# unitaryfoundation/qrack

Measured on NVIDIA H100. Metric: gates/sec at 30q random circuit; Apply2x2 HBM GB/s vs roofline, higher is better.
Workload: dtype f32

## Files before the change

### include/b200sv.h

```cpp
#ifndef B200SV_H
#define B200SV_H

#include <stddef.h>
#include <stdint.h>

#ifdef __cplusplus
extern "C" {
#endif

#define B200SV_OK 0
#define B200SV_EINVAL (-1)
#define B200SV_ENOMEM (-2)
#define B200SV_ECUDA (-3)
#define B200SV_ESTATE (-4)

typedef struct b200sv_state* b200sv_t;

int b200sv_abi_version(void);
const char* b200sv_last_error(void);
int b200sv_device_count(int* count);
int b200sv_device_info(int dev, uint64_t* total_bytes, uint64_t* free_bytes, int* sm_count);
int b200sv_can_access_peer(int dev, int peer, int* can);

int b200sv_create(int device, int n_qubits, int precision, b200sv_t* out);
// ... 91 lines not shown
int b200sv_indexed(b200sv_t s, int kind, int index_start, int index_length, int value_start, int value_length,
    int carry_index, int carry_in, const unsigned char* values);
int b200sv_hash(b200sv_t s, int start, int length, const unsigned char* values);
int b200sv_phase_flip_if_less(b200sv_t s, uint64_t greater_perm, int start, int length, int flag_index);

int b200sv_apply_gates(b200sv_t s, int n_gates, const uint64_t* off1, const uint64_t* off2, const uint64_t* pmasks,
    const double* mats8);

int b200sv_emulate_fused(int n_qubits, int precision, int n_gates, const uint64_t* off1, const uint64_t* off2,
    const uint64_t* pmasks, const double* mats8, void* host_state);
int b200sv_plan_gates(int n_qubits, int precision, int n_gates, const uint64_t* off1, const uint64_t* off2,
    const uint64_t* pmasks, const double* mats8, int* n_sweeps, int* n_passes, int* n_ops);
int b200sv_emulate_fused_pull(int n_qubits, int precision, int n_gates, const uint64_t* off1, const uint64_t* off2,
    const uint64_t* pmasks, const double* mats8, int k, const int* victim_bits, int rank, void* const* src_states,
    void* out_state);

typedef struct b200sv_stats {
    uint64_t gates_submitted;
    uint64_t kernel_launches;
    uint64_t fused_sweeps;
    uint64_t fused_gates;
    uint64_t single_launches;
    uint64_t bytes_swept;
    uint64_t pull_sweeps;
} b200sv_stats;
int b200sv_get_stats(b200sv_t s, b200sv_stats* out);
int b200sv_reset_stats(b200sv_t s);

int b200sv_timer_begin(b200sv_t s);
int b200sv_timer_end(b200sv_t s, double* elapsed_ms);
int b200sv_flush_l2(b200sv_t s, uint64_t bytes);

#ifdef __cplusplus
}
#endif
#endif
```

### qrack_b200/_abi.py

```python
from __future__ import annotations

import ctypes
import os
import subprocess
from ctypes import POINTER, c_char_p, c_double, c_int, c_uint64, c_void_p

_HERE = os.path.dirname(os.path.abspath(__file__))
LIB_PATH = os.environ.get("B200SV_LIB") or os.path.join(_HERE, "libb200sv.so")
CSRC = os.path.join(_HERE, "csrc")
SOURCES = ["b200sv.cu", "fused.cu"]
NVCC_FLAGS = ["-gencode", "arch=compute_90a,code=sm_90a", "-lineinfo", "-O3", "-std=c++17", "-Xcompiler", "-fPIC,-ffp-contract=off",
              "-shared", "-cudart", "static"]

B200SV_OK, B200SV_EINVAL, B200SV_ENOMEM, B200SV_ECUDA, B200SV_ESTATE = 0, -1, -2, -3, -4


class Stats(ctypes.Structure):
    _fields_ = [("gates_submitted", c_uint64), ("kernel_launches", c_uint64), ("fused_sweeps", c_uint64),
                ("fused_gates", c_uint64), ("single_launches", c_uint64), ("bytes_swept", c_uint64),
                ("pull_sweeps", c_uint64)]


H = c_void_p
SIGNATURES = {
    "b200sv_abi_version": [],
    "b200sv_device_count": [POINTER(c_int)],
    "b200sv_device_info": [c_int, POINTER(c_uint64), POINTER(c_uint64), POINTER(c_int)],
    "b200sv_can_access_peer": [c_int, c_int, POINTER(c_int)],
    "b200sv_create": [c_int, c_int, c_int, POINTER(H)],
    "b200sv_destroy": [H],
    "b200sv_clone": [H, POINTER(H)],
    "b200sv_qubit_count": [H, POINTER(c_int)],
    "b200sv_precision": [H, POINTER(c_int)],
    "b200sv_device": [H, POINTER(c_int)],
    "b200sv_set_device": [H, c_int],
# ... 64 lines not shown
    "b200sv_incdecsc": [H, c_uint64, c_int, c_int, c_int, c_int],
    "b200sv_muldiv": [H, c_int, c_uint64, c_int, c_int, c_int, c_uint64],
    "b200sv_modnout": [H, c_int, c_uint64, c_uint64, c_int, c_int, c_int, c_uint64],
    "b200sv_indexed": [H, c_int, c_int, c_int, c_int, c_int, c_int, c_int, c_char_p],
    "b200sv_hash": [H, c_int, c_int, c_char_p],
    "b200sv_phase_flip_if_less": [H, c_uint64, c_int, c_int, c_int],
    "b200sv_flush": [H],
    "b200sv_finish": [H],
    "b200sv_set_fusion": [H, c_int],
    "b200sv_emulate_fused": [c_int, c_int, c_int, POINTER(c_uint64), POINTER(c_uint64), POINTER(c_uint64), POINTER(c_double),
                             c_void_p],
    "b200sv_plan_gates": [c_int, c_int, c_int, POINTER(c_uint64), POINTER(c_uint64), POINTER(c_uint64), POINTER(c_double),
                          POINTER(c_int), POINTER(c_int), POINTER(c_int)],
    "b200sv_emulate_fused_pull": [c_int, c_int, c_int, POINTER(c_uint64), POINTER(c_uint64), POINTER(c_uint64), POINTER(c_double),
                                  c_int, POINTER(c_int), c_int, POINTER(c_void_p), c_void_p],
    "b200sv_get_stats": [H, POINTER(Stats)],
    "b200sv_reset_stats": [H],
    "b200sv_timer_begin": [H],
    "b200sv_timer_end": [H, POINTER(c_double)],
    "b200sv_flush_l2": [H, c_uint64],
}

_lib = None


def build(force: bool = False, verbose: bool = False) -> str:
    srcs = [os.path.join(CSRC, s) for s in SOURCES]
    deps = srcs + [os.path.join(CSRC, f) for f in os.listdir(CSRC) if f.endswith((".cuh", ".h", ".inl"))]
    deps.append(os.path.join(_HERE, "..", "include", "b200sv.h"))
    if not force and os.path.exists(LIB_PATH):
# ... 61 lines not shown
```

### qrack_b200/csrc/b200sv.cu

```cuda
#include "sv_common.cuh"

#include <type_traits>

#include <math.h>
#include <stdio.h>
#include <string.h>

#include <algorithm>
#include <map>
#include <mutex>

namespace b200sv {

static thread_local std::string g_err;
void set_error(const std::string& msg) { g_err = msg; }
int cuda_fail(cudaError_t e, const char* what)
{
    g_err = std::string(what) + ": " + cudaGetErrorString(e);
    cudaGetLastError();
    return (e == cudaErrorMemoryAllocation) ? B200SV_ENOMEM : B200SV_ECUDA;
}
static int einval(const char* msg)
{
    g_err = msg;
// ... 1291 lines not shown
    return B200SV_OK;
}

template <typename F> static int scratch_reduce(State* s, int k, F&& launch)
{
    SV_CUDA(cudaMemsetAsync(s->d_scratch, 0, k * sizeof(double), s->stream));
    launch();
    SV_TRY(launched(s));
    return read_scratch(s, k);
}

template <typename R>
static int launch_apply2x2(State* s, uint64_t off1, uint64_t off2, const double* m8, int nb, const uint64_t* pows, double nrm, double thresh,
    double* normOutDev);

static int run_gate_unfused(State* s, const GateOp& g)
{
    uint64_t pows[64];
    int nb = 0;
    const uint64_t pmask = g.cmask | (1ULL << g.target);
    for (uint64_t m = pmask; m; m &= m - 1U) {
        pows[nb++] = m & (~m + 1U);
    }
    const uint64_t off1 = g.cval, off2 = g.cval | (1ULL << g.target);
    return with_prec(s, [&](auto r) { return launch_apply2x2<decltype(r)>(s, off1, off2, g.m, nb, pows, 1.0, 0.0, nullptr); });
}

int launch_pull_gather(State* s)
{
    if (!s->pullPending) {
        return B200SV_OK;
// ... 10 lines not shown
    }
    a.vmask = s->pull.vmask >> apcLog;
    a.rankDep = s->pull.rankDep >> apcLog;
    const uint64_t nChunks = (s->dim() * s->amp_bytes()) / 16U;
    const unsigned grid = stream_grid(s->dev, (nChunks + 3) / 4, 256);
    k_exchange_gather<<<grid, 256, 0, s->stream>>>((uint4*)s->pull.out, nChunks, a);
    SV_TRY(launched(s));
    s->amps = s->pull.out;
    s->pullPending = false;
    return B200SV_OK;
}

static void drop_pending(State* s)
{
    s->queue.clear();
    if (s->pullPending) {
        s->amps = s->pull.out;
        s->pullPending = false;
    }
}

static int flush_queue(State* s)
{
    if (s->queue.empty()) {
        return s->pullPending ? launch_pull_gather(s) : B200SV_OK;
    }
    std::vector<GateOp> saved;
    const bool keep = s->queue.size() <= 8192;
    if (keep) {
        saved = s->queue;
// ... 842 lines not shown
        if (norm_out) {
            *norm_out = 0;
        }
        return B200SV_OK;
    }
    s->stats.gates_submitted++;
    const uint64_t diff = off1 ^ off2;
    if (!norm_out && s->fusion && diff && !(diff & (diff - 1U))) {
        GateOp g;
        make_gate_op(s->prec, off1, off2, pmask, m8, nrm, g);
        if (fused_accepts(s, g)) {
            s->queue.push_back(g);
            if (s->queue.size() >= 4096) {
                SV_TRY(flush_queue(s));
            }
            return B200SV_OK;
        }
    }
    SV_TRY(flush_queue(s));
    double* dn = nullptr;
    if (norm_out) {
        dn = s->d_scratch;
        SV_CUDA(cudaMemsetAsync(dn, 0, sizeof(double), s->stream));
    }
    SV_TRY(with_prec(s, [&](auto r) {
        return launch_apply2x2<decltype(r)>(s, off1, off2, m8, bit_count, pows, nrm, norm_thresh, dn);
    }));
    if (norm_out) {
        SV_TRY(read_scratch(s, 1));
        *norm_out = s->h_scratch[0];
    }
// ... 12 lines not shown
            return einval("apply_gates: every gate must be a single-target Apply2x2 form within the qubit bounds");
        }
    }
    if (!s->amps) {
        return B200SV_OK;
    }
    for (int i = 0; i < n_gates; ++i) {
        GateOp g;
        make_gate_op(s->prec, off1[i], off2[i], pmasks[i], mats8 + 8 * (size_t)i, 1.0, g);
        s->stats.gates_submitted++;
        if (s->fusion && fused_accepts(s, g)) {
            s->queue.push_back(g);
            if (s->queue.size() >= 4096) {
                SV_TRY(flush_queue(s));
            }
            continue;
        }
        SV_TRY(flush_queue(s));
        SV_TRY(run_gate_unfused(s, g));
    }
    return B200SV_OK;
}

int b200sv_xmask(b200sv_t s, uint64_t mask)
{
    SV_ENTER(s);
    if (mask >= s->dim()) {
        return einval("XMask mask out-of-bounds!");
    }
    if (!s->amps || !mask) {
// ... 916 lines not shown
        return einval("DecomposeDispose range is out-of-bounds!");
    }
    if (!length) {
        return B200SV_OK;
    }
    if (s->external || (dest && dest->external)) {
        return einval("Decompose on an external buffer");
    }
    if (dest && (dest->prec != s->prec || dest->nq != length)) {
        return einval("Decompose: destination size/precision mismatch");
    }
    SV_TRY(flush_queue(s));
    if (dest) {
        DevGuard g2(dest->dev);
        dest->queue.clear();
    }
    const int nl = s->nq - length;
    if (!s->amps) {
        s->nq = nl;
        if (dest) {
            SV_TRY(b200sv_zero(dest));
        }
        return B200SV_OK;
    }
    if (!nl) {
        if (dest) {
            if (dest->dev != s->dev) {
                SV_TRY(b200sv_copy_page(dest, s, 0, 0, s->dim()));
                free_amps(s);
            } else {
// ... 163 lines not shown
    if (n_gates < 0 || (n_gates && (!off1 || !off2 || !pmasks || !mats8)) || (precision != 32 && precision != 64) || n_qubits < 5 ||
        n_qubits > 62 || !n_sweeps || !n_passes || !n_ops) {
        return einval("plan_gates: bad arguments");
    }
    std::vector<GateOp> q((size_t)n_gates);
    for (int i = 0; i < n_gates; ++i) {
        const uint64_t diff = off1[i] ^ off2[i];
        if (!diff || (diff & (diff - 1U)) || (n_qubits < 64 && (pmasks[i] >> n_qubits)) || ((off1[i] | off2[i]) & ~pmasks[i])) {
            return einval("plan_gates: not a single-target gate");
        }
        make_gate_op(precision, off1[i], off2[i], pmasks[i], mats8 + 8 * (size_t)i, 1.0, q[(size_t)i]);
    }
    return fused_plan_gates(n_qubits, precision, q, n_sweeps, n_passes, n_ops);
}

int b200sv_emulate_fused(int n_qubits, int precision, int n_gates, const uint64_t* off1, const uint64_t* off2, const uint64_t* pmasks,
    const double* mats8, void* host_state)
{
    if (n_gates < 0 || (n_gates && (!off1 || !off2 || !pmasks || !mats8)) || !host_state || (precision != 32 && precision != 64) ||
        n_qubits < 5 || n_qubits > 30) {
        return einval("emulate_fused: bad arguments");
    }
    std::vector<GateOp> q((size_t)n_gates);
    const uint64_t dim = 1ULL << n_qubits;
    for (int i = 0; i < n_gates; ++i) {
        const uint64_t diff = off1[i] ^ off2[i];
        if (!diff || (diff & (diff - 1U)) || pmasks[i] >= dim || ((off1[i] | off2[i]) & ~pmasks[i])) {
            return einval("emulate_fused: not a single-target gate");
        }
        make_gate_op(precision, off1[i], off2[i], pmasks[i], mats8 + 8 * (size_t)i, 1.0, q[(size_t)i]);
    }
    return fused_emulate(n_qubits, precision, q, host_state);
}

int b200sv_emulate_fused_pull(int n_qubits, int precision, int n_gates, const uint64_t* off1, const uint64_t* off2,
    const uint64_t* pmasks, const double* mats8, int k, const int* victim_bits, int rank, void* const* src_states, void* out_state)
{
    if (n_gates < 0 || (n_gates && (!off1 || !off2 || !pmasks || !mats8)) || (precision != 32 && precision != 64) || n_qubits < 5 ||
        n_qubits > 30) {
        return einval("emulate_fused_pull: bad arguments");
    }
    PullArgs pa;
    SV_TRY(fill_pull_args(n_qubits, precision, k, victim_bits, rank, src_states, out_state, &pa));
    std::vector<GateOp> q((size_t)n_gates);
    const uint64_t dim = 1ULL << n_qubits;
    for (int i = 0; i < n_gates; ++i) {
        const uint64_t diff = off1[i] ^ off2[i];
// ... 31 lines not shown
```

### qrack_b200/csrc/fused.cu

```cuda
#include "sv_common.cuh"

#include <algorithm>
#include <atomic>
#include <cstdio>
#include <cstdlib>
#include <cstring>
#include <memory>
#include <mutex>

namespace b200sv {

constexpr int FUSED_KC = 12;
constexpr int FUSED_NT = 256;
constexpr int FUSED_RB = 4;
constexpr int FUSED_MINB = 2;
constexpr int FUSED_L = 6;

constexpr int MAX_HIGH = 8;
constexpr int MAX_PASS = 8;
constexpr int MAX_OPS = 96;
constexpr int MAX_HOST_OPS = 384;
constexpr int MAX_SLOTS = 128;
constexpr int MAX_NCH = 16;
constexpr int MAX_NA = 32;
// ... 728 lines not shown
            stage_out<R>(tilePsi, tileB, rowOff, nChunk, lcb, colMask, tid);
        }
    }
}

struct HostOp {
    int kind;
    int tq;
    uint64_t cmask;
    uint64_t cval;
    double m[8];
};

static inline uint64_t bitq(int q) { return 1ULL << q; }

static uint64_t rewrite_ops(std::vector<HostOp>& ops);
static uint64_t lower_queue(const std::vector<GateOp>& q, std::vector<HostOp>& out)
{
    out.clear();
    out.reserve(q.size() * 2);
    for (const GateOp& g : q) {
        HostOp h;
        memset(&h, 0, sizeof(h));
        if (g.kind == 1) {
            const bool one0 = (g.m[0] == 1.0 && g.m[1] == 0.0), one3 = (g.m[6] == 1.0 && g.m[7] == 0.0);
            const double n0 = g.m[0] * g.m[0] + g.m[1] * g.m[1];
            if (!one0 && n0 > 0.0) {
                h.kind = OP_PHASE;
                h.tq = -1;
                h.cmask = g.cmask;
                h.cval = g.cval;
                h.m[0] = g.m[0];
// ... 31 lines not shown
        }
        h.tq = g.target;
        h.cmask = g.cmask;
        h.cval = g.cval;
        memcpy(h.m, g.m, sizeof(h.m));
        const bool allReal = (g.m[1] == 0.0 && g.m[3] == 0.0 && g.m[5] == 0.0 && g.m[7] == 0.0);
        if (g.kind == 2 && g.m[2] == 1.0 && g.m[3] == 0.0 && g.m[4] == 1.0 && g.m[5] == 0.0) {
            h.kind = OP_XSWAP;
        } else if (!g.cmask && allReal && g.m[0] > 0.0 && g.m[0] == g.m[2] && g.m[0] == g.m[4] && g.m[6] == -g.m[0]) {
            h.kind = OP_HAD;
        } else {
            h.kind = OP_GENERAL;
        }
        out.push_back(h);
    }
    const uint64_t xtail = rewrite_ops(out);
    if (getenv("B200SV_FUSED_DEBUG")) {
        int cnt[5] = { 0, 0, 0, 0, 0 };
        for (const HostOp& h : out) {
            cnt[h.kind]++;
        }
        fprintf(stderr, "lowered: %zu gates -> %zu ops (general %d, hadamard %d, xswap %d, phase %d, rotation %d)\n", q.size(), out.size(), cnt[0],
            cnt[1], cnt[2], cnt[3], cnt[4]);
        if (atoi(getenv("B200SV_FUSED_DEBUG")) >= 2) {
            for (const HostOp& h : out) {
                fprintf(stderr, "   %s t=%d cmask=%llx cval=%llx m0=(%.3f,%.3f)\n", h.kind == OP_PHASE ? "PH" : (h.kind == OP_HAD ? "H " : (h.kind == OP_XSWAP ? "X " : (h.kind == OP_ROT ? "R " : "G "))),
                    h.tq, (unsigned long long)h.cmask, (unsigned long long)h.cval, h.m[0], h.m[1]);
            }
        }
    }
    return xtail;
// ... 13 lines not shown
                const double bx = b[2 * (2 * k + j)], by = b[2 * (2 * k + j) + 1];
                re += ax * bx - ay * by;
                im += ax * by + ay * bx;
            }
            r.m[2 * (2 * i + j)] = re;
            r.m[2 * (2 * i + j) + 1] = im;
        }
    }
    return r;
}
static inline bool is_had_form(const double* m)
{
    return m[1] == 0.0 && m[3] == 0.0 && m[5] == 0.0 && m[7] == 0.0 && m[0] > 0.0 && m[0] == m[2] && m[0] == m[4] && m[6] == -m[0];
}

static uint64_t rewrite_ops(std::vector<HostOp>& ops)
{
    std::vector<HostOp> out;
    std::vector<char> alive;
    out.reserve(ops.size() * 3);
    alive.reserve(ops.size() * 3);
    std::vector<int> hist[64];
    double gx = 1.0, gy = 0.0;
    auto touches = [](const HostOp& h) { return h.cmask | (h.tq >= 0 ? bitq(h.tq) : 0ULL); };
    auto push = [&](const HostOp& h) {
        const int idx = (int)out.size();
        out.push_back(h);
        alive.push_back(1);
        for (uint64_t m = touches(h); m; m &= m - 1U) {
            hist[__builtin_ctzll(m)].push_back(idx);
        }
// ... 154 lines not shown
            z.m[0] = -1.0;
            push(z);
            emit_u1(op.tq, HM);
        } else if (is_u1(op)) {
            emit_u1(op.tq, op.m);
        } else if (op.kind == OP_PHASE && op.cmask && !(op.cmask & (op.cmask - 1U))) {
            emit_phase1(__builtin_ctzll(op.cmask), op.cval ? 1 : 0, op.m[0], op.m[1]);
        } else if (op.kind == OP_PHASE && !op.cmask) {
            const double nx = gx * op.m[0] - gy * op.m[1];
            gy = gx * op.m[1] + gy * op.m[0];
            gx = nx;
        } else {
            push(op);
        }
    }
    uint64_t xtail = 0;
    if (__builtin_popcountll(xpend) > 4) {
        xtail = xpend;
    } else {
        for (uint64_t m = xpend; m; m &= m - 1U) {
            emit_bare_x(__builtin_ctzll(m));
        }
    }
    std::vector<HostOp> res;
    res.reserve(out.size() + 1);
    for (size_t i = 0; i < out.size(); ++i) {
        if (!alive[i]) {
            continue;
        }
        const HostOp& h = out[i];
        if (h.kind == OP_GENERAL && !h.cmask) {
            const double* m = h.m;
            const double n00 = m[0] * m[0] + m[1] * m[1], n10 = m[4] * m[4] + m[5] * m[5];
            const double n01 = m[2] * m[2] + m[3] * m[3], n11 = m[6] * m[6] + m[7] * m[7];
            const double ox = m[0] * m[2] + m[1] * m[3] + m[4] * m[6] + m[5] * m[7], oy = m[0] * m[3] - m[1] * m[2] + m[4] * m[7] - m[5] * m[6];
            if (fabs(n00 + n10 - 1.0) < 1e-5 && fabs(n01 + n11 - 1.0) < 1e-5 && fabs(ox) < 1e-5 && fabs(oy) < 1e-5 && n10 > 1e-24 && n01 > 1e-24) {
                const double c = sqrt(n00), sn = sqrt(n10);
                double g0x = 1.0, g0y = 0.0;
                if (c > 1e-12) {
                    g0x = m[0] / c;
                    g0y = m[1] / c;
// ... 20 lines not shown
                memset(&r, 0, sizeof(r));
                r.kind = OP_ROT;
                r.tq = h.tq;
                r.m[0] = c;
                r.m[1] = sm;
                res.push_back(r);
                if (ax != 1.0 || ay != 0.0) {
                    ph.m[0] = ax;
                    ph.m[1] = ay;
                    res.push_back(ph);
                }
                continue;
            }
        }
        res.push_back(h);
    }
    if (gx != 1.0 || gy != 0.0) {
        HostOp h;
        memset(&h, 0, sizeof(h));
        h.kind = OP_PHASE;
        h.tq = -1;
        h.m[0] = gx;
        h.m[1] = gy;
        res.push_back(h);
    }
    ops.swap(res);
    return xtail;
}

struct TileCfg {
// ... 765 lines not shown
            }
            buf.resize(mark);
            cfg.maxOps = cfg.maxOps * 3 / 4;
            continue;
        }
        window.insert(window.end(), pending.begin() + wsz, pending.end());
        pending.swap(window);
        *bytesOut = bytes;
        *scratchOut = scratch;
        *nOpsOut = sp.nOps;
        *nPassOut = (int)sp.passes.size();
        return B200SV_OK;
    }
}

struct Seg {
    size_t off, bytes, scratch, nops;
    int npass;
};

static int plan_list(std::vector<HostOp>& pending, const TileCfg& cfg, int prec, std::vector<unsigned char>& buf, std::vector<Seg>& segs)
{
    while (!pending.empty()) {
        const size_t off = buf.size();
        size_t bytes = 0, scratch = 0, nops = 0;
        int npass = 0;
        SV_TRY(plan_and_encode(pending, cfg, prec, buf, &bytes, &scratch, &nops, &npass));
        segs.push_back({ off, bytes, scratch, nops, npass });
        if (getenv("B200SV_FUSED_DEBUG")) {
            fprintf(stderr, "  program %zu B + scratch %zu B\n", bytes, scratch);
        }
    }
    return B200SV_OK;
}

struct Arena {
    unsigned char* dev = nullptr;
    unsigned char* host = nullptr;
    size_t cap = 0;
    cudaEvent_t done = nullptr;
    bool pending = false;
};
static std::vector<std::pair<State*, std::unique_ptr<Arena>>>& arenas()
{
    static std::vector<std::pair<State*, std::unique_ptr<Arena>>> a;
    return a;
}
static std::mutex& arena_mutex()
{
    static std::mutex m;
    return m;
}
static Arena* get_arena(State* s)
{
    std::lock_guard<std::mutex> lk(arena_mutex());
    for (auto& kv : arenas()) {
// ... 13 lines not shown
        for (size_t i = 0; i < v.size(); ++i) {
            if (v[i].first == s) {
                mine = std::move(v[i].second);
                v.erase(v.begin() + i);
                break;
            }
        }
    }
    if (mine) {
        if (mine->dev) {
            cudaFree(mine->dev);
        }
        if (mine->host) {
            cudaFreeHost(mine->host);
        }
        if (mine->done) {
            cudaEventDestroy(mine->done);
        }
    }
}

bool fused_accepts(const State* s, const GateOp&) { return s->nq >= 5 && s->nq <= 62; }

template <typename R, int VAR, bool PULL = false>
static int launch_sweep_v(State* s, const unsigned char* dprog, uint32_t progBytes, uint32_t scratchBytes, uint64_t nTiles)
{
    auto kern = k_fused_sweep<R, VAR, PULL>;
    const size_t shm = ((size_t)16 << FUSED_KC) + progBytes + scratchBytes;
    static std::atomic<unsigned long long> attr_set_mask{ 0 };
    if (!(attr_set_mask.load() & (1ULL << s->dev))) {
        SV_CUDA(cudaFuncSetAttribute(kern, cudaFuncAttributeMaxDynamicSharedMemorySize, (int)(((size_t)16 << FUSED_KC) + MAX_PROG_BYTES_2CTA)));
        attr_set_mask.fetch_or(1ULL << s->dev);
    }
    const uint64_t maxGrid = (uint64_t)sm_count(s->dev) * FUSED_MINB;
// ... 4 lines not shown
    if (PULL) {
        s->amps = s->pull.out;
        s->pullPending = false;
    }
    return B200SV_OK;
}

template <typename R>
static int launch_sweep(State* s, const unsigned char* dprog, uint32_t progBytes, uint32_t scratchBytes, uint64_t nTiles, int var)
{
    return var == 2 ? launch_sweep_v<R, 2>(s, dprog, progBytes, scratchBytes, nTiles)
                    : (var == 1 ? launch_sweep_v<R, 1>(s, dprog, progBytes, scratchBytes, nTiles)
                                : launch_sweep_v<R, 0>(s, dprog, progBytes, scratchBytes, nTiles));
}

int fused_flush(State* s)
{
    if (s->queue.empty()) {
        return s->pullPending ? launch_pull_gather(s) : B200SV_OK;
    }
    if (!s->amps) {
        s->queue.clear();
        return B200SV_OK;
    }
    std::vector<HostOp> pending;
    const uint64_t xtail = lower_queue(s->queue, pending);
    const size_t nGates = s->queue.size();
    const TileCfg cfg = make_cfg(s->nq, s->prec);
    std::vector<unsigned char> buf;
    std::vector<Seg> segs;
    SV_TRY(plan_list(pending, cfg, s->prec, buf, segs));
    s->queue.clear();
    if (s->pullPending && segs.empty()) {
        SV_TRY(launch_pull_gather(s));
    }
    if (segs.empty()) {
        return xtail ? launch_xmask(s, xtail) : B200SV_OK;
    }
    Arena* ar = get_arena(s);
    if (!ar->done) {
        SV_CUDA(cudaEventCreateWithFlags(&ar->done, cudaEventDisableTiming));
    }
    const uint64_t nTiles = s->dim() >> cfg.kA;
    if (ar->pending) {
        SV_CUDA(cudaEventSynchronize(ar->done));
        ar->pending = false;
    }
    if (ar->cap < buf.size()) {
        if (ar->dev) {
            cudaFree(ar->dev);
            cudaFreeHost(ar->host);
        }
        ar->cap = std::max<size_t>(buf.size() * 2, 1 << 20);
        SV_CUDA(cudaMalloc(&ar->dev, ar->cap));
        SV_CUDA(cudaMallocHost(&ar->host, ar->cap));
    }
    memcpy(ar->host, buf.data(), buf.size());
    SV_CUDA(cudaMemcpyAsync(ar->dev, ar->host, buf.size(), cudaMemcpyHostToDevice, s->stream));
    for (size_t i = 0; i < segs.size(); ++i) {
        const unsigned char* dp = ar->dev + segs[i].off;
        const uint32_t pb = (uint32_t)segs[i].bytes, sb = (uint32_t)segs[i].scratch;
        const DevSweep* dsw = reinterpret_cast<const DevSweep*>(buf.data() + segs[i].off);
        const bool full = dsw->needFull != 0;
        const int var = full ? 2 : (dsw->nRot ? 1 : 0);
        if (s->pullPending) {
            if (s->prec == 32) {
                SV_TRY((launch_sweep_v<float, 2, true>(s, dp, pb, sb, nTiles)));
            } else {
                SV_TRY((launch_sweep_v<double, 2, true>(s, dp, pb, sb, nTiles)));
            }
            s->stats.pull_sweeps++;
        } else if (s->prec == 32) {
            SV_TRY(launch_sweep<float>(s, dp, pb, sb, nTiles, var));
        } else {
            SV_TRY(launch_sweep<double>(s, dp, pb, sb, nTiles, var));
        }
        s->stats.kernel_launches++;
        s->stats.fused_sweeps++;
        s->stats.bytes_swept += 2ULL * s->dim() * s->amp_bytes();
    }
    s->stats.fused_gates += nGates;
    SV_CUDA(cudaEventRecord(ar->done, s->stream));
    ar->pending = true;
    if (xtail) {
        SV_TRY(launch_xmask(s, xtail));
    }
    return B200SV_OK;
}

template <typename R> struct EmuC {
    R x, y;
};
template <typename R> static inline EmuC<R> emu_mul(EmuC<R> a, R px, R py) { return EmuC<R>{ a.x * px - a.y * py, a.x * py + a.y * px }; }

template <typename R>
static void emu_exec_op(std::vector<EmuC<R>>& a, const DevOp<R>& op, uint32_t xsb, const R* tileScale, int NA,
    const DevMember<R>* members, const uint2* eff, const R* rotTab)
{
    const uint32_t code = op.code, emask = op.emask, lmaskSb = op.lmaskSb, lvalSb = op.lvalSb;
    bool tp = true;
    if (code & CODE_HAS_SB) {
        tp = (xsb & lmaskSb) == lvalSb;
// ... 253 lines not shown
                        }
                    }
                }
            }
        }
        if (!sw.directOut) {
            for (uint32_t c = 0; c < nChunk; ++c) {
                for (int w = 0; w < APC; ++w) {
                    tilePsi[rowOff[c >> lcb] + (uint64_t)(c & colMask) * APC + w] = tile[(size_t)swz(c) * APC + w];
                }
            }
        }
    }
}

int fused_emulate(int n_qubits, int precision, const std::vector<GateOp>& q, void* host_state, const PullArgs* pull)
{
    std::vector<HostOp> pending;
    const uint64_t xtail = lower_queue(q, pending);
    const TileCfg cfg = make_cfg(n_qubits, precision);
    std::vector<unsigned char> buf;
    std::vector<Seg> segs;
    SV_TRY(plan_list(pending, cfg, precision, buf, segs));
    if (pull && segs.empty()) {
        const uint64_t dim = 1ULL << n_qubits;
        for (uint64_t i = 0; i < dim; ++i) {
            if (precision == 32) {
                reinterpret_cast<EmuC<float>*>(host_state)[i] = emu_pull_load<float>(*pull, i);
            } else {
                reinterpret_cast<EmuC<double>*>(host_state)[i] = emu_pull_load<double>(*pull, i);
            }
        }
        pull = nullptr;
    }
    for (const Seg& sg : segs) {
        if (precision == 32) {
            emulate_sweep<float>(buf.data() + sg.off, reinterpret_cast<EmuC<float>*>(host_state), n_qubits, cfg, pull);
        } else {
            emulate_sweep<double>(buf.data() + sg.off, reinterpret_cast<EmuC<double>*>(host_state), n_qubits, cfg, pull);
        }
        pull = nullptr;
    }
    if (xtail) {
        const uint64_t dim = 1ULL << n_qubits;
        const size_t ab = (precision == 32) ? 8 : 16;
        unsigned char* st = reinterpret_cast<unsigned char*>(host_state);
        unsigned char tmp[16];
        for (uint64_t i = 0; i < dim; ++i) {
            const uint64_t j = i ^ xtail;
            if (i < j) {
                memcpy(tmp, st + i * ab, ab);
                memcpy(st + i * ab, st + j * ab, ab);
                memcpy(st + j * ab, tmp, ab);
            }
        }
    }
    return B200SV_OK;
}

int fused_plan_gates(int n_qubits, int precision, const std::vector<GateOp>& q, int* n_sweeps, int* n_passes, int* n_ops)
{
    std::vector<HostOp> pending;
    (void)lower_queue(q, pending);
    const TileCfg cfg = make_cfg(n_qubits, precision);
    int sweeps = 0, passes = 0, ops = 0;
    std::vector<unsigned char> buf;
    while (!pending.empty()) {
        size_t bytes = 0, nops = 0, scratch = 0;
        int npass = 0;
        buf.clear();
        SV_TRY(plan_and_encode(pending, cfg, precision, buf, &bytes, &scratch, &nops, &npass));
        ++sweeps;
// ... 11 lines not shown
```

### qrack_b200/csrc/sv_common.cuh

```cuda
#pragma once

#include <cuda_runtime.h>
#include <stdint.h>

#include <string>
#include <vector>

#include "../../include/b200sv.h"

namespace b200sv {

template <typename R> struct Cx;
template <> struct Cx<float> {
    typedef float2 type;
};
template <> struct Cx<double> {
    typedef double2 type;
};

template <typename R> __host__ __device__ __forceinline__ typename Cx<R>::type mk(R re, R im)
{
    typename Cx<R>::type c;
    c.x = re;
    c.y = im;
// ... 91 lines not shown

#define SV_TRY(call)                                                                                                   \
    do {                                                                                                               \
        int r__ = (call);                                                                                              \
        if (r__ != B200SV_OK)                                                                                          \
            return r__;                                                                                                \
    } while (0)

int sm_count(int dev);

int fused_flush(State* s);
int launch_xmask(State* s, uint64_t mask);
bool fused_accepts(const State* s, const GateOp& g);
void fused_release(State* s);
int launch_pull_gather(State* s);
int fused_emulate(int n_qubits, int precision, const std::vector<GateOp>& q, void* host_state, const PullArgs* pull = nullptr);
int fused_plan_gates(int n_qubits, int precision, const std::vector<GateOp>& q, int* n_sweeps, int* n_passes, int* n_ops);

}

struct b200sv_state : public b200sv::State {};
```

Before: 5537.

## Plan and launch fused sweeps early while gates are still being queued

As gates are enqueued, the queue is periodically re-lowered and any prefix whose ops are final gets planned and launched as fused sweeps before the flush. The goal is to overlap host-side planning with GPU execution and cut flush latency. Program upload moves to a ring of pinned/device buffers with per-slot events and a separate copy stream. The cost is repeated lowering of the growing queue, more complex state (a carry that must match at flush), and a fallback to unfused gates when planning fails mid-stream.

```diff
diff --git a/include/b200sv.h b/include/b200sv.h
--- a/include/b200sv.h
+++ b/include/b200sv.h
@@ -129,6 +129,11 @@
 int b200sv_emulate_fused_pull(int n_qubits, int precision, int n_gates, const uint64_t* off1, const uint64_t* off2,
     const uint64_t* pmasks, const double* mats8, int k, const int* victim_bits, int rank, void* const* src_states,
     void* out_state);
+int b200sv_emulate_fused_fail_at(int n_qubits, int precision, int n_gates, const uint64_t* off1, const uint64_t* off2,
+    const uint64_t* pmasks, const double* mats8, int fail_at_sweep, void* host_state);
+int b200sv_encode_fused(int n_qubits, int precision, int n_gates, const uint64_t* off1, const uint64_t* off2,
+    const uint64_t* pmasks, const double* mats8, int step, unsigned char* out, uint64_t capacity, uint64_t* n_bytes,
+    int* n_sweeps);
 
 typedef struct b200sv_stats {
     uint64_t gates_submitted;
@@ -138,6 +143,10 @@
     uint64_t single_launches;
     uint64_t bytes_swept;
     uint64_t pull_sweeps;
+    uint64_t fused_flushes;
+    uint64_t plan_ns;
+    uint64_t first_sweep_ns;
+    uint64_t early_sweeps;
 } b200sv_stats;
 int b200sv_get_stats(b200sv_t s, b200sv_stats* out);
 int b200sv_reset_stats(b200sv_t s);
diff --git a/qrack_b200/_abi.py b/qrack_b200/_abi.py
--- a/qrack_b200/_abi.py
+++ b/qrack_b200/_abi.py
@@ -18,7 +18,7 @@
 class Stats(ctypes.Structure):
     _fields_ = [("gates_submitted", c_uint64), ("kernel_launches", c_uint64), ("fused_sweeps", c_uint64),
                 ("fused_gates", c_uint64), ("single_launches", c_uint64), ("bytes_swept", c_uint64),
-                ("pull_sweeps", c_uint64)]
+                ("pull_sweeps", c_uint64), ("fused_flushes", c_uint64), ("plan_ns", c_uint64), ("first_sweep_ns", c_uint64), ("early_sweeps", c_uint64)]
 
 
 H = c_void_p
@@ -113,6 +113,10 @@
                           POINTER(c_int), POINTER(c_int), POINTER(c_int)],
     "b200sv_emulate_fused_pull": [c_int, c_int, c_int, POINTER(c_uint64), POINTER(c_uint64), POINTER(c_uint64), POINTER(c_double),
                                   c_int, POINTER(c_int), c_int, POINTER(c_void_p), c_void_p],
+    "b200sv_emulate_fused_fail_at": [c_int, c_int, c_int, POINTER(c_uint64), POINTER(c_uint64), POINTER(c_uint64),
+                                     POINTER(c_double), c_int, c_void_p],
+    "b200sv_encode_fused": [c_int, c_int, c_int, POINTER(c_uint64), POINTER(c_uint64), POINTER(c_uint64), POINTER(c_double),
+                            c_int, c_void_p, c_uint64, POINTER(c_uint64), POINTER(c_int)],
     "b200sv_get_stats": [H, POINTER(Stats)],
     "b200sv_reset_stats": [H],
     "b200sv_timer_begin": [H],
diff --git a/qrack_b200/csrc/b200sv.cu b/qrack_b200/csrc/b200sv.cu
--- a/qrack_b200/csrc/b200sv.cu
+++ b/qrack_b200/csrc/b200sv.cu
@@ -1329,7 +1329,7 @@
 static int launch_apply2x2(State* s, uint64_t off1, uint64_t off2, const double* m8, int nb, const uint64_t* pows, double nrm, double thresh,
     double* normOutDev);
 
-static int run_gate_unfused(State* s, const GateOp& g)
+int run_gate_unfused(State* s, const GateOp& g)
 {
     uint64_t pows[64];
     int nb = 0;
@@ -1370,6 +1370,7 @@
 static void drop_pending(State* s)
 {
     s->queue.clear();
+    fused_drop(s);
     if (s->pullPending) {
         s->amps = s->pull.out;
         s->pullPending = false;
@@ -2242,7 +2243,7 @@
             if (s->queue.size() >= 4096) {
                 SV_TRY(flush_queue(s));
             }
-            return B200SV_OK;
+            return fused_advance(s);
         }
     }
     SV_TRY(flush_queue(s));
@@ -2285,6 +2286,7 @@
             if (s->queue.size() >= 4096) {
                 SV_TRY(flush_queue(s));
             }
+            SV_TRY(fused_advance(s));
             continue;
         }
         SV_TRY(flush_queue(s));
@@ -3231,6 +3233,7 @@
     if (dest) {
         DevGuard g2(dest->dev);
         dest->queue.clear();
+        fused_drop(dest);
     }
     const int nl = s->nq - length;
     if (!s->amps) {
@@ -3424,23 +3427,60 @@
     return fused_plan_gates(n_qubits, precision, q, n_sweeps, n_passes, n_ops);
 }
 
-int b200sv_emulate_fused(int n_qubits, int precision, int n_gates, const uint64_t* off1, const uint64_t* off2, const uint64_t* pmasks,
-    const double* mats8, void* host_state)
-{
-    if (n_gates < 0 || (n_gates && (!off1 || !off2 || !pmasks || !mats8)) || !host_state || (precision != 32 && precision != 64) ||
-        n_qubits < 5 || n_qubits > 30) {
-        return einval("emulate_fused: bad arguments");
-    }
-    std::vector<GateOp> q((size_t)n_gates);
+static int host_hook_gates(const char* who, int n_qubits, int precision, int n_gates, const uint64_t* off1, const uint64_t* off2,
+    const uint64_t* pmasks, const double* mats8, std::vector<GateOp>& q)
+{
+    if (n_gates < 0 || (n_gates && (!off1 || !off2 || !pmasks || !mats8)) || (precision != 32 && precision != 64) || n_qubits < 5 ||
+        n_qubits > 30) {
+        return einval((std::string(who) + ": bad arguments").c_str());
+    }
+    q.resize((size_t)n_gates);
     const uint64_t dim = 1ULL << n_qubits;
     for (int i = 0; i < n_gates; ++i) {
         const uint64_t diff = off1[i] ^ off2[i];
         if (!diff || (diff & (diff - 1U)) || pmasks[i] >= dim || ((off1[i] | off2[i]) & ~pmasks[i])) {
-            return einval("emulate_fused: not a single-target gate");
+            return einval((std::string(who) + ": not a single-target gate").c_str());
         }
         make_gate_op(precision, off1[i], off2[i], pmasks[i], mats8 + 8 * (size_t)i, 1.0, q[(size_t)i]);
     }
-    return fused_emulate(n_qubits, precision, q, host_state);
+    return B200SV_OK;
+}
+
+int b200sv_emulate_fused(int n_qubits, int precision, int n_gates, const uint64_t* off1, const uint64_t* off2, const uint64_t* pmasks,
+    const double* mats8, void* host_state)
+{
+    return b200sv_emulate_fused_fail_at(n_qubits, precision, n_gates, off1, off2, pmasks, mats8, -1, host_state);
+}
+
+int b200sv_emulate_fused_fail_at(int n_qubits, int precision, int n_gates, const uint64_t* off1, const uint64_t* off2,
+    const uint64_t* pmasks, const double* mats8, int fail_at_sweep, void* host_state)
+{
+    if (!host_state) {
+        return einval("emulate_fused: null state");
+    }
+    std::vector<GateOp> q;
+    SV_TRY(host_hook_gates("emulate_fused", n_qubits, precision, n_gates, off1, off2, pmasks, mats8, q));
+    return fused_emulate(n_qubits, precision, q, host_state, nullptr, fail_at_sweep);
+}
+
+int b200sv_encode_fused(int n_qubits, int precision, int n_gates, const uint64_t* off1, const uint64_t* off2, const uint64_t* pmasks,
+    const double* mats8, int step, unsigned char* out, uint64_t capacity, uint64_t* n_bytes, int* n_sweeps)
+{
+    if (!n_bytes || !n_sweeps) {
+        return einval("encode_fused: null out pointer");
+    }
+    std::vector<GateOp> q;
+    SV_TRY(host_hook_gates("encode_fused", n_qubits, precision, n_gates, off1, off2, pmasks, mats8, q));
+    std::vector<unsigned char> progs;
+    SV_TRY(fused_encode(n_qubits, precision, q, step, progs, n_sweeps));
+    *n_bytes = progs.size();
+    if (out) {
+        if (capacity < progs.size()) {
+            return einval("encode_fused: output buffer too small");
+        }
+        memcpy(out, progs.data(), progs.size());
+    }
+    return B200SV_OK;
 }
 
 int b200sv_emulate_fused_pull(int n_qubits, int precision, int n_gates, const uint64_t* off1, const uint64_t* off2,
diff --git a/qrack_b200/csrc/fused.cu b/qrack_b200/csrc/fused.cu
--- a/qrack_b200/csrc/fused.cu
+++ b/qrack_b200/csrc/fused.cu
@@ -2,6 +2,7 @@
 
 #include <algorithm>
 #include <atomic>
+#include <chrono>
 #include <cstdio>
 #include <cstdlib>
 #include <cstring>
@@ -766,8 +767,8 @@
 
 static inline uint64_t bitq(int q) { return 1ULL << q; }
 
-static uint64_t rewrite_ops(std::vector<HostOp>& ops);
-static uint64_t lower_queue(const std::vector<GateOp>& q, std::vector<HostOp>& out)
+static uint64_t rewrite_ops(std::vector<HostOp>& ops, size_t* finalOut);
+static uint64_t lower_queue(const std::vector<GateOp>& q, std::vector<HostOp>& out, size_t* finalOut = nullptr)
 {
     out.clear();
     out.reserve(q.size() * 2);
@@ -829,7 +830,7 @@
         }
         out.push_back(h);
     }
-    const uint64_t xtail = rewrite_ops(out);
+    const uint64_t xtail = rewrite_ops(out, finalOut);
     if (getenv("B200SV_FUSED_DEBUG")) {
         int cnt[5] = { 0, 0, 0, 0, 0 };
         for (const HostOp& h : out) {
@@ -873,7 +874,7 @@
     return m[1] == 0.0 && m[3] == 0.0 && m[5] == 0.0 && m[7] == 0.0 && m[0] > 0.0 && m[0] == m[2] && m[0] == m[4] && m[6] == -m[0];
 }
 
-static uint64_t rewrite_ops(std::vector<HostOp>& ops)
+static uint64_t rewrite_ops(std::vector<HostOp>& ops, size_t* finalOut)
 {
     std::vector<HostOp> out;
     std::vector<char> alive;
@@ -1058,6 +1059,18 @@
             push(op);
         }
     }
+    size_t firstOpen = out.size();
+    if (finalOut) {
+        for (int b = 0; b < 64; ++b) {
+            for (size_t k = hist[b].size(); k-- > 0;) {
+                const int idx = hist[b][k];
+                if (__builtin_popcountll(touches(out[(size_t)idx])) > 1) {
+                    break;
+                }
+                firstOpen = std::min(firstOpen, (size_t)idx);
+            }
+        }
+    }
     uint64_t xtail = 0;
     if (__builtin_popcountll(xpend) > 4) {
         xtail = xpend;
@@ -1069,6 +1082,9 @@
     std::vector<HostOp> res;
     res.reserve(out.size() + 1);
     for (size_t i = 0; i < out.size(); ++i) {
+        if (finalOut && i == firstOpen) {
+            *finalOut = res.size();
+        }
         if (!alive[i]) {
             continue;
         }
@@ -1119,6 +1135,9 @@
             }
         }
         res.push_back(h);
+    }
+    if (finalOut && firstOpen >= out.size()) {
+        *finalOut = res.size();
     }
     if (gx != 1.0 || gy != 0.0) {
         HostOp h;
@@ -1914,32 +1933,148 @@
     }
 }
 
-struct Seg {
-    size_t off, bytes, scratch, nops;
-    int npass;
-};
-
-static int plan_list(std::vector<HostOp>& pending, const TileCfg& cfg, int prec, std::vector<unsigned char>& buf, std::vector<Seg>& segs)
-{
-    while (!pending.empty()) {
-        const size_t off = buf.size();
+static GateOp host_op_gate(const HostOp& h)
+{
+    GateOp g;
+    memset(&g, 0, sizeof(g));
+    g.cmask = h.cmask;
+    g.cval = h.cval;
+    if (h.kind == OP_PHASE) {
+        const int t = h.cmask ? __builtin_ctzll(h.cmask) : 0;
+        g.target = t;
+        g.cmask &= ~bitq(t);
+        g.cval &= ~bitq(t);
+        g.kind = 1;
+        g.m[0] = g.m[6] = 1.0;
+        const bool on0 = !h.cmask || !(h.cval & bitq(t)), on1 = !h.cmask || (h.cval & bitq(t));
+        if (on0) {
+            g.m[0] = h.m[0];
+            g.m[1] = h.m[1];
+        }
+        if (on1) {
+            g.m[6] = h.m[0];
+            g.m[7] = h.m[1];
+        }
+    } else if (h.kind == OP_ROT) {
+        g.target = h.tq;
+        g.m[0] = g.m[6] = h.m[0];
+        g.m[2] = -h.m[1];
+        g.m[4] = h.m[1];
+    } else {
+        g.target = h.tq;
+        memcpy(g.m, h.m, sizeof(g.m));
+    }
+    return g;
+}
+
+template <typename SweepFn, typename GateFn>
+static int run_sweeps(std::vector<HostOp>& pending, const TileCfg& cfg, int prec, int first, int failAt, uint64_t* planNs,
+    SweepFn&& sweep, GateFn&& gate)
+{
+    std::vector<unsigned char> prog;
+    for (int i = first; !pending.empty(); ++i) {
+        prog.clear();
         size_t bytes = 0, scratch = 0, nops = 0;
         int npass = 0;
-        SV_TRY(plan_and_encode(pending, cfg, prec, buf, &bytes, &scratch, &nops, &npass));
-        segs.push_back({ off, bytes, scratch, nops, npass });
+        const auto t0 = std::chrono::steady_clock::now();
+        int rc = B200SV_ESTATE;
+        if (i == failAt) {
+            set_error("fused planner failure injected by the test hook");
+        } else {
+            rc = plan_and_encode(pending, cfg, prec, prog, &bytes, &scratch, &nops, &npass);
+        }
+        if (planNs) {
+            *planNs += (uint64_t)std::chrono::duration_cast<std::chrono::nanoseconds>(std::chrono::steady_clock::now() - t0).count();
+        }
+        if (rc != B200SV_OK) {
+            if (i == 0 || rc != B200SV_ESTATE) {
+                return rc;
+            }
+            for (const HostOp& h : pending) {
+                SV_TRY(gate(host_op_gate(h)));
+            }
+            pending.clear();
+            return B200SV_OK;
+        }
         if (getenv("B200SV_FUSED_DEBUG")) {
             fprintf(stderr, "  program %zu B + scratch %zu B\n", bytes, scratch);
         }
+        SV_TRY(sweep(prog.data(), bytes, scratch, i));
     }
     return B200SV_OK;
 }
 
+struct Carry {
+    std::vector<HostOp> fed;
+    std::vector<HostOp> pending;
+    int swept = 0;
+    size_t triedAt = 0;
+    bool stop = false;
+};
+constexpr size_t EARLY_FROM = 512, EARLY_EVERY = 128;
+
+template <typename SweepFn>
+static int advance(Carry& c, const std::vector<GateOp>& q, const TileCfg& cfg, int prec, uint64_t* planNs, SweepFn&& sweep)
+{
+    const auto t0 = std::chrono::steady_clock::now();
+    std::vector<HostOp> low;
+    size_t fin = 0;
+    (void)lower_queue(q, low, &fin);
+    if (fin > c.fed.size()) {
+        c.pending.insert(c.pending.end(), low.begin() + (long)c.fed.size(), low.begin() + (long)fin);
+        c.fed.insert(c.fed.end(), low.begin() + (long)c.fed.size(), low.begin() + (long)fin);
+    }
+    if (planNs) {
+        *planNs += (uint64_t)std::chrono::duration_cast<std::chrono::nanoseconds>(std::chrono::steady_clock::now() - t0).count();
+    }
+    std::vector<unsigned char> prog;
+    while (!c.stop && c.pending.size() >= PLAN_WINDOW) {
+        prog.clear();
+        size_t bytes = 0, scratch = 0, nops = 0;
+        int npass = 0;
+        const auto t1 = std::chrono::steady_clock::now();
+        const int rc = plan_and_encode(c.pending, cfg, prec, prog, &bytes, &scratch, &nops, &npass);
+        if (planNs) {
+            *planNs += (uint64_t)std::chrono::duration_cast<std::chrono::nanoseconds>(std::chrono::steady_clock::now() - t1).count();
+        }
+        if (rc != B200SV_OK) {
+            c.stop = true;
+            break;
+        }
+        SV_TRY(sweep(prog.data(), bytes, scratch, c.swept));
+        ++c.swept;
+    }
+    return B200SV_OK;
+}
+
+static int resume(Carry& c, const std::vector<GateOp>& q, std::vector<HostOp>& pending, int* first, uint64_t* xtail)
+{
+    std::vector<HostOp> low;
+    *xtail = lower_queue(q, low);
+    const bool same = low.size() >= c.fed.size() && (c.fed.empty() || !memcmp(low.data(), c.fed.data(), c.fed.size() * sizeof(HostOp)));
+    if (!same && c.swept) {
+        c = Carry();
+        set_error("fused flush: the sweeps planned early do not begin the queue's plan (state undefined)");
+        return B200SV_EINVAL;
+    }
+    const size_t skip = same ? c.fed.size() : 0;
+    pending = same ? std::move(c.pending) : std::vector<HostOp>();
+    pending.insert(pending.end(), low.begin() + (long)skip, low.end());
+    *first = c.swept;
+    c = Carry();
+    return B200SV_OK;
+}
+
+constexpr int PROG_RING = 32;
 struct Arena {
     unsigned char* dev = nullptr;
     unsigned char* host = nullptr;
-    size_t cap = 0;
-    cudaEvent_t done = nullptr;
-    bool pending = false;
+    cudaStream_t copy = nullptr;
+    cudaEvent_t loaded[PROG_RING] = {};
+    cudaEvent_t done[PROG_RING] = {};
+    bool busy[PROG_RING] = {};
+    int next = 0;
+    Carry carry;
 };
 static std::vector<std::pair<State*, std::unique_ptr<Arena>>>& arenas()
 {
@@ -1983,10 +2118,40 @@
         if (mine->host) {
             cudaFreeHost(mine->host);
         }
-        if (mine->done) {
-            cudaEventDestroy(mine->done);
-        }
-    }
+        for (int k = 0; k < PROG_RING; ++k) {
+            if (mine->loaded[k]) {
+                cudaEventDestroy(mine->loaded[k]);
+            }
+            if (mine->done[k]) {
+                cudaEventDestroy(mine->done[k]);
+            }
+        }
+        if (mine->copy) {
+            cudaStreamDestroy(mine->copy);
+        }
+    }
+}
+
+static int arena_ready(Arena* ar)
+{
+    if (!ar->copy) {
+        SV_CUDA(cudaStreamCreateWithFlags(&ar->copy, cudaStreamNonBlocking));
+    }
+    for (int k = 0; k < PROG_RING; ++k) {
+        if (!ar->loaded[k]) {
+            SV_CUDA(cudaEventCreateWithFlags(&ar->loaded[k], cudaEventDisableTiming));
+        }
+        if (!ar->done[k]) {
+            SV_CUDA(cudaEventCreateWithFlags(&ar->done[k], cudaEventDisableTiming));
+        }
+    }
+    if (!ar->host) {
+        SV_CUDA(cudaMallocHost(&ar->host, PROG_RING * MAX_PROG_BYTES_2CTA));
+    }
+    if (!ar->dev) {
+        SV_CUDA(cudaMalloc(&ar->dev, PROG_RING * MAX_PROG_BYTES_2CTA));
+    }
+    return B200SV_OK;
 }
 
 bool fused_accepts(const State* s, const GateOp&) { return s->nq >= 5 && s->nq <= 62; }
@@ -2021,78 +2186,110 @@
                                 : launch_sweep_v<R, 0>(s, dprog, progBytes, scratchBytes, nTiles));
 }
 
+static int launch_program(State* s, Arena* ar, const unsigned char* prog, size_t bytes, size_t scratch)
+{
+    SV_TRY(arena_ready(ar));
+    const int k = ar->next;
+    ar->next = (k + 1) % PROG_RING;
+    if (ar->busy[k]) {
+        SV_CUDA(cudaEventSynchronize(ar->done[k]));
+        ar->busy[k] = false;
+    }
+    unsigned char* hp = ar->host + (size_t)k * MAX_PROG_BYTES_2CTA;
+    unsigned char* dp = ar->dev + (size_t)k * MAX_PROG_BYTES_2CTA;
+    memcpy(hp, prog, bytes);
+    SV_CUDA(cudaMemcpyAsync(dp, hp, bytes, cudaMemcpyHostToDevice, ar->copy));
+    SV_CUDA(cudaEventRecord(ar->loaded[k], ar->copy));
+    SV_CUDA(cudaStreamWaitEvent(s->stream, ar->loaded[k], 0));
+    const uint64_t nTiles = s->dim() >> make_cfg(s->nq, s->prec).kA;
+    const uint32_t pb = (uint32_t)bytes, sb = (uint32_t)scratch;
+    const DevSweep* dsw = reinterpret_cast<const DevSweep*>(prog);
+    const bool full = dsw->needFull != 0;
+    const int var = full ? 2 : (dsw->nRot ? 1 : 0);
+    if (s->pullPending) {
+        if (s->prec == 32) {
+            SV_TRY((launch_sweep_v<float, 2, true>(s, dp, pb, sb, nTiles)));
+        } else {
+            SV_TRY((launch_sweep_v<double, 2, true>(s, dp, pb, sb, nTiles)));
+        }
+        s->stats.pull_sweeps++;
+    } else if (s->prec == 32) {
+        SV_TRY(launch_sweep<float>(s, dp, pb, sb, nTiles, var));
+    } else {
+        SV_TRY(launch_sweep<double>(s, dp, pb, sb, nTiles, var));
+    }
+    SV_CUDA(cudaEventRecord(ar->done[k], s->stream));
+    ar->busy[k] = true;
+    s->stats.kernel_launches++;
+    s->stats.fused_sweeps++;
+    s->stats.bytes_swept += 2ULL * s->dim() * s->amp_bytes();
+    return B200SV_OK;
+}
+
+int fused_advance(State* s)
+{
+    if (!s->amps || s->queue.size() < EARLY_FROM) {
+        return B200SV_OK;
+    }
+    Arena* ar = get_arena(s);
+    Carry& c = ar->carry;
+    if (c.stop || s->queue.size() < c.triedAt + EARLY_EVERY) {
+        return B200SV_OK;
+    }
+    c.triedAt = s->queue.size();
+    return advance(c, s->queue, make_cfg(s->nq, s->prec), s->prec, &s->stats.plan_ns,
+        [&](const unsigned char* prog, size_t bytes, size_t scratch, int) {
+            SV_TRY(launch_program(s, ar, prog, bytes, scratch));
+            s->stats.early_sweeps++;
+            return B200SV_OK;
+        });
+}
+
+void fused_drop(State* s) { get_arena(s)->carry = Carry(); }
+
 int fused_flush(State* s)
 {
     if (s->queue.empty()) {
         return s->pullPending ? launch_pull_gather(s) : B200SV_OK;
     }
+    Arena* ar = get_arena(s);
     if (!s->amps) {
         s->queue.clear();
+        ar->carry = Carry();
         return B200SV_OK;
     }
+    const auto t0 = std::chrono::steady_clock::now();
     std::vector<HostOp> pending;
-    const uint64_t xtail = lower_queue(s->queue, pending);
+    uint64_t xtail = 0;
+    int swept = 0;
+    SV_TRY(resume(ar->carry, s->queue, pending, &swept, &xtail));
     const size_t nGates = s->queue.size();
     const TileCfg cfg = make_cfg(s->nq, s->prec);
-    std::vector<unsigned char> buf;
-    std::vector<Seg> segs;
-    SV_TRY(plan_list(pending, cfg, s->prec, buf, segs));
+    s->stats.fused_flushes++;
+    s->stats.plan_ns += (uint64_t)std::chrono::duration_cast<std::chrono::nanoseconds>(std::chrono::steady_clock::now() - t0).count();
+    const int early = swept;
+    auto sweep = [&](const unsigned char* prog, size_t bytes, size_t scratch, int) -> int {
+        SV_TRY(launch_program(s, ar, prog, bytes, scratch));
+        if (!swept) {
+            s->stats.first_sweep_ns +=
+                (uint64_t)std::chrono::duration_cast<std::chrono::nanoseconds>(std::chrono::steady_clock::now() - t0).count();
+        }
+        ++swept;
+        return B200SV_OK;
+    };
+    const int rc = run_sweeps(pending, cfg, s->prec, early, -1, &s->stats.plan_ns, sweep,
+        [&](const GateOp& g) { return run_gate_unfused(s, g); });
+    if (rc != B200SV_OK && !swept) {
+        return rc;
+    }
     s->queue.clear();
-    if (s->pullPending && segs.empty()) {
+    SV_TRY(rc);
+    if (swept) {
+        s->stats.fused_gates += nGates;
+    } else if (s->pullPending) {
         SV_TRY(launch_pull_gather(s));
     }
-    if (segs.empty()) {
-        return xtail ? launch_xmask(s, xtail) : B200SV_OK;
-    }
-    Arena* ar = get_arena(s);
-    if (!ar->done) {
-        SV_CUDA(cudaEventCreateWithFlags(&ar->done, cudaEventDisableTiming));
-    }
-    const uint64_t nTiles = s->dim() >> cfg.kA;
-    if (ar->pending) {
-        SV_CUDA(cudaEventSynchronize(ar->done));
-        ar->pending = false;
-    }
-    if (ar->cap < buf.size()) {
-        if (ar->dev) {
-            cudaFree(ar->dev);
-            cudaFreeHost(ar->host);
-        }
-        ar->cap = std::max<size_t>(buf.size() * 2, 1 << 20);
-        SV_CUDA(cudaMalloc(&ar->dev, ar->cap));
-        SV_CUDA(cudaMallocHost(&ar->host, ar->cap));
-    }
-    memcpy(ar->host, buf.data(), buf.size());
-    SV_CUDA(cudaMemcpyAsync(ar->dev, ar->host, buf.size(), cudaMemcpyHostToDevice, s->stream));
-    for (size_t i = 0; i < segs.size(); ++i) {
-        const unsigned char* dp = ar->dev + segs[i].off;
-        const uint32_t pb = (uint32_t)segs[i].bytes, sb = (uint32_t)segs[i].scratch;
-        const DevSweep* dsw = reinterpret_cast<const DevSweep*>(buf.data() + segs[i].off);
-        const bool full = dsw->needFull != 0;
-        const int var = full ? 2 : (dsw->nRot ? 1 : 0);
-        if (s->pullPending) {
-            if (s->prec == 32) {
-                SV_TRY((launch_sweep_v<float, 2, true>(s, dp, pb, sb, nTiles)));
-            } else {
-                SV_TRY((launch_sweep_v<double, 2, true>(s, dp, pb, sb, nTiles)));
-            }
-            s->stats.pull_sweeps++;
-        } else if (s->prec == 32) {
-            SV_TRY(launch_sweep<float>(s, dp, pb, sb, nTiles, var));
-        } else {
-            SV_TRY(launch_sweep<double>(s, dp, pb, sb, nTiles, var));
-        }
-        s->stats.kernel_launches++;
-        s->stats.fused_sweeps++;
-        s->stats.bytes_swept += 2ULL * s->dim() * s->amp_bytes();
-    }
-    s->stats.fused_gates += nGates;
-    SV_CUDA(cudaEventRecord(ar->done, s->stream));
-    ar->pending = true;
-    if (xtail) {
-        SV_TRY(launch_xmask(s, xtail));
-    }
-    return B200SV_OK;
+    return xtail ? launch_xmask(s, xtail) : B200SV_OK;
 }
 
 template <typename R> struct EmuC {
@@ -2376,15 +2573,51 @@
     }
 }
 
-int fused_emulate(int n_qubits, int precision, const std::vector<GateOp>& q, void* host_state, const PullArgs* pull)
+template <typename R> static void emu_apply_gate(EmuC<R>* psi, int nq, const GateOp& g)
+{
+    R m[8];
+    for (int k = 0; k < 8; ++k) {
+        m[k] = (R)g.m[k];
+    }
+    const uint64_t tb = bitq(g.target), pmask = g.cmask | tb;
+    for (uint64_t i = 0; i < (1ULL << nq); ++i) {
+        if ((i & pmask) == g.cval) {
+            const EmuC<R> x = psi[i], y = psi[i | tb];
+            const EmuC<R> x0 = emu_mul(x, m[0], m[1]), y1 = emu_mul(y, m[2], m[3]);
+            const EmuC<R> x2 = emu_mul(x, m[4], m[5]), y3 = emu_mul(y, m[6], m[7]);
+            psi[i] = EmuC<R>{ x0.x + y1.x, x0.y + y1.y };
+            psi[i | tb] = EmuC<R>{ x2.x + y3.x, x2.y + y3.y };
+        }
+    }
+}
+
+int fused_emulate(int n_qubits, int precision, const std::vector<GateOp>& q, void* host_state, const PullArgs* pull, int failAt)
 {
     std::vector<HostOp> pending;
     const uint64_t xtail = lower_queue(q, pending);
     const TileCfg cfg = make_cfg(n_qubits, precision);
-    std::vector<unsigned char> buf;
-    std::vector<Seg> segs;
-    SV_TRY(plan_list(pending, cfg, precision, buf, segs));
-    if (pull && segs.empty()) {
+    int swept = 0;
+    SV_TRY(run_sweeps(
+        pending, cfg, precision, 0, failAt, nullptr,
+        [&](const unsigned char* prog, size_t, size_t, int) {
+            if (precision == 32) {
+                emulate_sweep<float>(prog, reinterpret_cast<EmuC<float>*>(host_state), n_qubits, cfg, pull);
+            } else {
+                emulate_sweep<double>(prog, reinterpret_cast<EmuC<double>*>(host_state), n_qubits, cfg, pull);
+            }
+            pull = nullptr;
+            ++swept;
+            return B200SV_OK;
+        },
+        [&](const GateOp& g) {
+            if (precision == 32) {
+                emu_apply_gate<float>(reinterpret_cast<EmuC<float>*>(host_state), n_qubits, g);
+            } else {
+                emu_apply_gate<double>(reinterpret_cast<EmuC<double>*>(host_state), n_qubits, g);
+            }
+            return B200SV_OK;
+        }));
+    if (pull && !swept) {
         const uint64_t dim = 1ULL << n_qubits;
         for (uint64_t i = 0; i < dim; ++i) {
             if (precision == 32) {
@@ -2393,15 +2626,6 @@
                 reinterpret_cast<EmuC<double>*>(host_state)[i] = emu_pull_load<double>(*pull, i);
             }
         }
-        pull = nullptr;
-    }
-    for (const Seg& sg : segs) {
-        if (precision == 32) {
-            emulate_sweep<float>(buf.data() + sg.off, reinterpret_cast<EmuC<float>*>(host_state), n_qubits, cfg, pull);
-        } else {
-            emulate_sweep<double>(buf.data() + sg.off, reinterpret_cast<EmuC<double>*>(host_state), n_qubits, cfg, pull);
-        }
-        pull = nullptr;
     }
     if (xtail) {
         const uint64_t dim = 1ULL << n_qubits;
@@ -2418,6 +2642,26 @@
         }
     }
     return B200SV_OK;
+}
+
+int fused_encode(int n_qubits, int precision, const std::vector<GateOp>& q, int step, std::vector<unsigned char>& out, int* n_sweeps)
+{
+    const TileCfg cfg = make_cfg(n_qubits, precision);
+    *n_sweeps = 0;
+    auto sweep = [&](const unsigned char* prog, size_t bytes, size_t, int) {
+        out.insert(out.end(), prog, prog + bytes);
+        ++*n_sweeps;
+        return B200SV_OK;
+    };
+    Carry c;
+    for (size_t n = (size_t)std::max(step, 0); step > 0 && n < q.size(); n += (size_t)step) {
+        SV_TRY(advance(c, std::vector<GateOp>(q.begin(), q.begin() + (long)n), cfg, precision, nullptr, sweep));
+    }
+    std::vector<HostOp> pending;
+    uint64_t xtail = 0;
+    int first = 0;
+    SV_TRY(resume(c, q, pending, &first, &xtail));
+    return run_sweeps(pending, cfg, precision, first, -1, nullptr, sweep, [](const GateOp&) { return B200SV_OK; });
 }
 
 int fused_plan_gates(int n_qubits, int precision, const std::vector<GateOp>& q, int* n_sweeps, int* n_passes, int* n_ops)
diff --git a/qrack_b200/csrc/sv_common.cuh b/qrack_b200/csrc/sv_common.cuh
--- a/qrack_b200/csrc/sv_common.cuh
+++ b/qrack_b200/csrc/sv_common.cuh
@@ -129,7 +129,12 @@
 bool fused_accepts(const State* s, const GateOp& g);
 void fused_release(State* s);
 int launch_pull_gather(State* s);
-int fused_emulate(int n_qubits, int precision, const std::vector<GateOp>& q, void* host_state, const PullArgs* pull = nullptr);
+int run_gate_unfused(State* s, const GateOp& g);
+int fused_emulate(int n_qubits, int precision, const std::vector<GateOp>& q, void* host_state, const PullArgs* pull = nullptr,
+    int failAt = -1);
+int fused_encode(int n_qubits, int precision, const std::vector<GateOp>& q, int step, std::vector<unsigned char>& out, int* n_sweeps);
+int fused_advance(State* s);
+void fused_drop(State* s);
 int fused_plan_gates(int n_qubits, int precision, const std::vector<GateOp>& q, int* n_sweeps, int* n_passes, int* n_ops);
 
 }
```

Result: faster. 5888 (median of 6 runs) (+6.3%).
